# sukui-genomics-cn/hmm_layer

Hardware: AMD Instinct MI355X
Metric: HMM cell-updates/sec (batch x len x states) fwd-bwd, 15-state model (higher is better)
Workload: dtype f32

## Files before the change

hmm_layer_amd/csrc/hmm_engine.hip:

```cpp

#include <hip/hip_runtime.h>
#include <stdint.h>
#include <stdlib.h>
#include <mutex>
#include <type_traits>
#include <vector>
#include "hmm_engine.h"

typedef float f4 __attribute__((ext_vector_type(4)));
typedef int i4 __attribute__((ext_vector_type(4)));

#ifndef HMM_REDUCE_PF
#define HMM_REDUCE_PF 8
#endif
#ifndef HMM_NT_STORE
#define HMM_NT_STORE 1
#endif
#ifndef HMM_PSI
#define HMM_PSI 1
#endif
#ifndef HMM_BWD_FULL
#define HMM_BWD_FULL 0
#endif
#ifndef HMM_FWD_PF2
// ... 46 lines not shown
    int k, b, L, q;
    int NB;
    int T, C;
    int nsub;
    long long nchains;
    int cpw;
    int seq_start;
    int G, gsize;
    size_t o_ops, o_exps, o_prefix, o_llpre, o_suffix, o_lsuf, o_ckpt, o_loglik, o_topo, total;
    size_t o_phi, o_nexact;
    size_t o_flags;
    size_t o_xend, o_rstart;
    size_t o_wtab, o_wlist, o_wcnt, o_dfix;
    size_t o_wshift;
    size_t o_upi;
    size_t o_gops, o_gexps, o_gprefix, o_gllpre, o_gsuffix, o_glsuf;
};

static size_t align_up(size_t x) { return (x + 255) & ~(size_t)255; }
#define PLAN_WIN_STRIDE 34
#define PLAN_WSH_STRIDE 24

static int choose_T(long long NB, int L) {
    {
        const int t = opt(HMM_OPT_CHUNK);
        if (t >= 16 && t <= MAX_T && t % 16 == 0) return t;
    }
    long long t = (NB * (long long)L) / 32768;
    long long tb = 16;
    while (tb * tb * tb * 4 < 9ll * L && tb < MAX_T) tb += 16;
    if (t < tb) t = tb;
    t = ((t + 16 - 1) / 16) * 16;
    if (t < 16) t = 16;
    if (t > MAX_T) t = MAX_T;
    long long lmax = (((long long)L + 16 - 1) / 16) * 16;
    if (t > lmax) t = lmax;
    return (int)t;
}

static int make_plan(int op, int k, int b, int L, int q, Plan *p, int T_fixed = 0) {
    if (k < 1 || b < 1 || L < 1 || q < 1) return HMM_ERR_BAD_SHAPE;
    if (q > QP) return HMM_ERR_Q_UNSUPPORTED;
    if ((long long)k * b > (1ll << 30) / 64) return HMM_ERR_BAD_SHAPE;
    p->k = k; p->b = b; p->L = L; p->q = q;
    p->NB = k * b;
    p->T = T_fixed ? T_fixed : choose_T(p->NB, L);
    p->C = (L + p->T - 1) / p->T;
    p->nsub = p->T / SUB;
    p->nchains = (long long)p->NB * p->C;
    p->cpw = 16;
    p->seq_start = 1;
    size_t off = 0;
    p->o_ops = off;    off = align_up(off + (size_t)p->nchains * QP * QP * sizeof(float));
    p->o_exps = off;   off = align_up(off + (size_t)p->nchains * QP * sizeof(int));
    p->o_prefix = off; off = align_up(off + (size_t)p->nchains * QP * sizeof(float));
    p->o_llpre = off;  off = align_up(off + (size_t)p->nchains * sizeof(double));
    p->o_suffix = off; off = align_up(off + (size_t)p->nchains * QP * sizeof(float));
    p->o_lsuf = off;   off = align_up(off + (size_t)p->nchains * sizeof(double));
    p->o_loglik = off; off = align_up(off + (size_t)p->NB * sizeof(double));
    p->o_topo = off;   off = align_up(off + (size_t)p->k * sizeof(int));
    p->o_phi = off;    off = align_up(off + (size_t)p->nchains * sizeof(float));
    p->o_nexact = off; off = align_up(off + sizeof(int));
    p->o_flags = off;  off = align_up(off + (size_t)p->NB * sizeof(int));
    p->o_xend = off;   off = align_up(off + (size_t)p->nchains * QP * sizeof(float));
    p->o_rstart = off; off = align_up(off + (size_t)p->nchains * QP * sizeof(float));
    p->o_wtab = off;   off = align_up(off + (size_t)p->NB * PLAN_WIN_STRIDE * sizeof(int));
    p->o_wlist = off;  off = align_up(off + (size_t)p->NB * sizeof(int));
    p->o_wcnt = off;   off = align_up(off + 4 * sizeof(int));
    p->o_dfix = off;   off = align_up(off + (size_t)p->NB * sizeof(double));
    p->o_wshift = off; off = align_up(off + ((op == HMM_OP_FORWARD || op == HMM_OP_BACKWARD) ? (size_t)p->NB * PLAN_WSH_STRIDE * sizeof(double) : 0));
    p->o_upi = off;    off = align_up(off + (size_t)p->k * p->q * sizeof(float));
    p->G = 0; p->gsize = 0;
    if (p->C >= SCAN2_MIN_C) {
        int gs = 1;
        while (gs * gs < p->C) ++gs;
        p->gsize = gs;
        p->G = (p->C + gs - 1) / gs;
    }
    const size_t ng = (size_t)p->NB * (p->G > 0 ? p->G : 1);
    p->o_gops = off;    off = align_up(off + ng * QP * QP * sizeof(float));
    p->o_gexps = off;   off = align_up(off + ng * QP * sizeof(int));
    p->o_gprefix = off; off = align_up(off + ng * QP * sizeof(float));
    p->o_gllpre = off;  off = align_up(off + ng * sizeof(double));
    p->o_gsuffix = off; off = align_up(off + ng * QP * sizeof(float));
    p->o_glsuf = off;   off = align_up(off + ng * sizeof(double));
    p->o_ckpt = off;
    if (op == HMM_OP_POSTERIOR) {
        const size_t scan_rows = (size_t)(((long long)p->b * p->C + 15) / 16) * 16 * p->nsub;
        const size_t exact_rows = (size_t)((p->b + 15) / 16) * 16 * (size_t)(((p->L + 15) / 16) * 16 / SUB);
        off = align_up(off + (size_t)p->k * (scan_rows > exact_rows ? scan_rows : exact_rows) * QP * sizeof(float));
    }
    p->total = off;
    return HMM_OK;
}

static int make_xplan(const Plan &p, Plan *x) {
    *x = p;
    x->T = ((p.L + 15) / 16) * 16;
    x->C = 1;
    x->nsub = x->T / SUB;
    x->nchains = p.NB;
    x->G = 0; x->gsize = 0;
    const long long seq_bytes = (long long)x->T * p.q * (long long)sizeof(float);
    x->cpw = 16 * seq_bytes < (1ll << 31) - 4096 ? 16 : 1;
    if (opt(HMM_OPT_EXACT) == HMM_EXACT_ALWAYS_NARROW) x->cpw = 1;
    if (seq_bytes >= (1ll << 31) - 4096) return HMM_ERR_BAD_SHAPE;
    return HMM_OK;
}


__device__ __forceinline__ f4 mfma4(const float (&a)[4], f4 x) {
    const f4 z = {0.f, 0.f, 0.f, 0.f};
    f4 d = __builtin_amdgcn_mfma_f32_16x16x4f32(a[0], x.x, z, 0, 0, 0);
    d = __builtin_amdgcn_mfma_f32_16x16x4f32(a[1], x.y, d, 0, 0, 0);
    d = __builtin_amdgcn_mfma_f32_16x16x4f32(a[2], x.z, d, 0, 0, 0);
    d = __builtin_amdgcn_mfma_f32_16x16x4f32(a[3], x.w, d, 0, 0, 0);
    return d;
}

__device__ __forceinline__ f4 mfma4v(f4 a, f4 x, f4 c) {
    c = __builtin_amdgcn_mfma_f32_16x16x4f32(a.x, x.x, c, 0, 0, 0);
    c = __builtin_amdgcn_mfma_f32_16x16x4f32(a.y, x.y, c, 0, 0, 0);
    c = __builtin_amdgcn_mfma_f32_16x16x4f32(a.z, x.z, c, 0, 0, 0);
    c = __builtin_amdgcn_mfma_f32_16x16x4f32(a.w, x.w, c, 0, 0, 0);
    return c;
}

__device__ __forceinline__ void swap16(float &a, float &b) {
    asm("s_nop 1\n\tv_permlane16_swap_b32_e32 %0, %1" : "+v"(a), "+v"(b));
}
__device__ __forceinline__ void swap32(float &a, float &b) {
    asm("s_nop 1\n\tv_permlane32_swap_b32_e32 %0, %1" : "+v"(a), "+v"(b));
}
__device__ __forceinline__ float col_sum(float v) {
    float a = v, b = v;
    swap16(a, b);
    a += b; b = a;
    swap32(a, b);
    return a + b;
}
__device__ __forceinline__ float col_max(float v) {
    float a = v, b = v;
    swap16(a, b);
    a = fmaxf(a, b); b = a;
    swap32(a, b);
    return fmaxf(a, b);
}
__device__ __forceinline__ float hsum(f4 v) { return (v.x + v.y) + (v.z + v.w); }
__device__ __forceinline__ float hmax(f4 v) { return fmaxf(fmaxf(v.x, v.y), fmaxf(v.z, v.w)); }

__device__ __forceinline__ __amdgpu_buffer_rsrc_t make_rsrc(const void *base, unsigned long long bytes) {
    unsigned n = bytes > 0xFFFFFFF0ull ? 0xFFFFFFF0u : (unsigned)bytes;
    return __builtin_amdgcn_make_buffer_rsrc((void *)base, 0, (int)n, 0x00020000);
}
template <int N>
__device__ __forceinline__ void ld_rows(__amdgpu_buffer_rsrc_t r, int voff, int rowb, f4 (&e)[N]) {
#pragma unroll
    for (int s = 0; s < N; ++s)
        e[s] = __builtin_bit_cast(f4, __builtin_amdgcn_raw_buffer_load_b128(r, voff + s * rowb, 0, HMM_LD_AUX));
}

struct Bounds { f4 lo, hi; };
__device__ __forceinline__ Bounds make_bounds(int g, int q, float eps) {
    Bounds bd;
    const float inf = __builtin_inff();
    bd.lo.x = (4 * g + 0 < q) ? eps : 0.f;  bd.hi.x = (4 * g + 0 < q) ? inf : 0.f;
    bd.lo.y = (4 * g + 1 < q) ? eps : 0.f;  bd.hi.y = (4 * g + 1 < q) ? inf : 0.f;
    bd.lo.z = (4 * g + 2 < q) ? eps : 0.f;  bd.hi.z = (4 * g + 2 < q) ? inf : 0.f;
    bd.lo.w = (4 * g + 3 < q) ? eps : 0.f;  bd.hi.w = (4 * g + 3 < q) ? inf : 0.f;
    return bd;
}
__device__ __forceinline__ f4 clampE(f4 e, const Bounds &bd) {
    f4 r;
    r.x = __builtin_amdgcn_fmed3f(e.x, bd.lo.x, bd.hi.x);
    r.y = __builtin_amdgcn_fmed3f(e.y, bd.lo.y, bd.hi.y);
    r.z = __builtin_amdgcn_fmed3f(e.z, bd.lo.z, bd.hi.z);
    r.w = __builtin_amdgcn_fmed3f(e.w, bd.lo.w, bd.hi.w);
    return r;
}
__device__ __forceinline__ f4 fmax4(f4 v, float s) {
    f4 r = {fmaxf(v.x, s), fmaxf(v.y, s), fmaxf(v.z, s), fmaxf(v.w, s)};
    return r;
}
__device__ __forceinline__ f4 sel4(bool c, f4 a, f4 b) { return c ? a : b; }

__device__ __forceinline__ void load_A(const float *A, int q, int g, int n, float (&af)[4], float (&ab)[4]) {
#pragma unroll
    for (int kk = 0; kk < 4; ++kk) {
        int s = 4 * g + kk;
        bool ok = (s < q) && (n < q);
        af[kk] = ok ? A[s * q + n] : 0.f;
        ab[kk] = ok ? A[n * q + s] : 0.f;
    }
}


__device__ __forceinline__ void reduce_chain(const float *__restrict__ A, const float *__restrict__ E,
                                             float *__restrict__ ops, int *__restrict__ exps,
                                             const int *__restrict__ topo, const Plan &p, float eps, long long chain) {
    const int lane = threadIdx.x & 63, g = lane >> 4, n = lane & 15;
    const int seq = (int)(chain / p.C), c = (int)(chain - (long long)seq * p.C);
    const int m = seq / p.b;
    if (topo && topo[m] != 0) return;
    const int t0 = c * p.T;
    const int len = min(p.T, p.L - t0);
    const int q = p.q;

    float af[4], ab[4];
    load_A(A + (size_t)m * q * q, q, g, n, af, ab);
    const Bounds bd = make_bounds(g, q, eps);

    const float *base = E + ((size_t)seq * p.L + t0) * q;
    const __amdgpu_buffer_rsrc_t rs = make_rsrc(base, (unsigned long long)len * q * sizeof(float));
    const int rowb = q * (int)sizeof(float);
    int voff = g * 16;

    f4 X;
    X.x = (4 * g + 0 == n) ? 1.f : 0.f;
    X.y = (4 * g + 1 == n) ? 1.f : 0.f;
    X.z = (4 * g + 2 == n) ? 1.f : 0.f;
    X.w = (4 * g + 3 == n) ? 1.f : 0.f;
    int ex = 0;

    auto rescale = [&](f4 &V) {
        float s = col_sum(hsum(V));
        int xe = __builtin_amdgcn_frexp_expf(s);
        float sc = __builtin_amdgcn_ldexpf(1.0f, -xe);
        V = V * sc;
        ex += xe;
    };

    int t = 0;
    if (c == 0 && p.seq_start) {
        f4 e0[1];
        ld_rows<1>(rs, voff, rowb, e0);
        X = X * clampE(e0[0], bd);
        rescale(X);
        voff += rowb;
        t = 1;
    }
    constexpr int PF = HMM_REDUCE_PF;
    f4 en[PF];
    ld_rows<PF>(rs, voff, rowb, en);
    for (; t < len; t += PF) {
        f4 ec[PF];
#pragma unroll
        for (int u = 0; u < PF; ++u) ec[u] = en[u];
        voff += PF * rowb;
        ld_rows<PF>(rs, voff, rowb, en);
#pragma unroll
        for (int u = 0; u < PF; ++u) {
            if (t + u < len) {
                X = mfma4(af, X) * clampE(ec[u], bd);
                rescale(X);
            }
        }
    }
    float *o = ops + (size_t)chain * QP * QP;
    o[(4 * g + 0) * QP + n] = X.x;
    o[(4 * g + 1) * QP + n] = X.y;
    o[(4 * g + 2) * QP + n] = X.z;
    o[(4 * g + 3) * QP + n] = X.w;
    if (g == 0) exps[(size_t)chain * QP + n] = ex;
}

__global__ __launch_bounds__(256) void k_reduce(const float *__restrict__ A, const float *__restrict__ E,
                                                float *__restrict__ ops, int *__restrict__ exps,
                                                const int *__restrict__ topo, Plan p, float eps) {
    const long long stride = (long long)gridDim.x * 4;
    for (long long chain = (long long)blockIdx.x * 4 + __builtin_amdgcn_readfirstlane(threadIdx.x >> 6);
         chain < p.nchains; chain += stride)
        reduce_chain(A, E, ops, exps, topo, p, eps, chain);
}



struct TopoGene15 {
    static constexpr int Q = 15, NE = 23, ID = 1;
    static constexpr int start[Q + 1] = {0, 2, 4, 6, 8, 10, 13, 15, 16, 17, 18, 19, 20, 21, 22, 23};
    static constexpr int src[NE] = {0, 14, 8, 1, 9, 2, 10, 3, 11, 6, 7, 4, 12, 5, 13, 0, 4, 5, 6, 1, 2, 3, 5};
};
struct TopoGene7 {
    static constexpr int Q = 7, NE = 15, ID = 2;
    static constexpr int start[Q + 1] = {0, 2, 4, 6, 8, 11, 13, 15};
    static constexpr int src[NE] = {0, 6, 4, 1, 5, 2, 6, 3, 0, 6, 3, 4, 1, 5, 2};
};

struct TopoGene29 {
    static constexpr int Q = 29, NE = 45, ID = 3;
    static constexpr int start[Q + 1] = {0, 3, 5, 7, 9, 11, 13, 15, 17, 19, 22, 25, 27, 29, 30, 31, 32, 33, 34, 35, 36,
                                         37, 38, 39, 40, 41, 42, 43, 44, 45};
    static constexpr int src[NE] = {0, 27, 28, 15, 1, 16, 2, 17, 3, 18, 4, 19, 5, 20, 6, 21, 11, 22, 12, 13, 7, 23, 14,
                                    8, 24, 9, 25, 10, 26, 0, 0, 7, 8, 9, 10, 11, 12, 1, 2, 3, 4, 5, 6, 9, 10};
};

template <class T>
__host__ __device__ constexpr int out_degree(int i) {
    int n = 0;
    for (int e = 0; e < T::NE; ++e) n += (T::src[e] == i) ? 1 : 0;
    return n;
}
#define TOPO_UNIT 16
template <class T>
__device__ __forceinline__ bool edge_in(int i, int j) {
    bool ok = false;
    for (int e = T::start[j]; e < T::start[j + 1]; ++e) ok = ok || (T::src[e] == i);
    return ok;
}

#define TOPO_EXACT 255
__global__ __launch_bounds__(64) void k_topo_check(const float *__restrict__ A, int *__restrict__ topo, int k, int q,
                                                   int force_dense, int exact_mode, float eps, int *__restrict__ nexact,
                                                   int *__restrict__ wcnt = nullptr) {
    const int m = blockIdx.x;
    const float *Am = A + (size_t)m * q * q;
    if (m == 0 && threadIdx.x == 0) *nexact = 0;
    if (m == 0 && threadIdx.x < 4 && wcnt) wcnt[threadIdx.x] = 0;
    bool exact = exact_mode == HMM_EXACT_ALWAYS || exact_mode == HMM_EXACT_ALWAYS_NARROW;
    if (exact_mode == HMM_EXACT_AUTO) {
        int row = 0;
        if ((int)threadIdx.x < q)
            for (int j = 0; j < q; ++j) row |= (Am[threadIdx.x * q + j] > eps) ? (1 << j) : 0;
        for (int it = 0; it < 8; ++it) {
            int nr = 0;
            for (int j = 0; j < q; ++j) {
                const int rj = __builtin_amdgcn_readlane(row, j);
                nr |= ((row >> j) & 1) ? rj : 0;
            }
            row = nr;
        }
        const bool notfull = (int)threadIdx.x < q && row != (1 << q) - 1;
        exact = __ballot(notfull) != 0ull;
    }
    if (exact) {
        if (threadIdx.x == 0) topo[m] = TOPO_EXACT;
        return;
    }
    bool bad15 = q != TopoGene15::Q, bad7 = q != TopoGene7::Q;
    bool nonunit15 = false, nonunit7 = false;
    if (!force_dense && (!bad15 || !bad7))
        for (int e = threadIdx.x; e < q * q; e += 64) {
            const float a = Am[e];
            const int i = e / q, j = e - i * q;
            if (!bad15) {
                const bool in = edge_in<TopoGene15>(i, j);
                bad15 = a != 0.f && !in;
                nonunit15 = nonunit15 || (in && a != 1.0f && out_degree<TopoGene15>(i) == 1);
            }
            if (!bad7) {
                const bool in = edge_in<TopoGene7>(i, j);
                bad7 = a != 0.f && !in;
                nonunit7 = nonunit7 || (in && a != 1.0f && out_degree<TopoGene7>(i) == 1);
            }
        }
    const bool any15 = __ballot(bad15) != 0ull, any7 = __ballot(bad7) != 0ull;
    const bool nu15 = __ballot(nonunit15) != 0ull, nu7 = __ballot(nonunit7) != 0ull;
    if (threadIdx.x == 0) {
        int id = force_dense ? 0 : (!any15 ? TopoGene15::ID : (!any7 ? TopoGene7::ID : 0));
        if (id == TopoGene15::ID && !nu15) id |= TOPO_UNIT;
        if (id == TopoGene7::ID && !nu7) id |= TOPO_UNIT;
        topo[m] = id;
    }
}

#define SP_TILE 16

#ifndef HMM_RS_AHEAD
#define HMM_RS_AHEAD 0
#endif
#ifndef HMM_RS_UNI
#define HMM_RS_UNI 1
#endif
#ifndef HMM_POST_BLOCK
#define HMM_POST_BLOCK 16
#endif
#ifndef HMM_RS_SUM2
#define HMM_RS_SUM2 1
#endif
#ifndef HMM_RS_WPE
#define HMM_RS_WPE 4
#endif
#if HMM_RS_WPE
#define RS_ATTR __attribute__((amdgpu_waves_per_eu(HMM_RS_WPE, HMM_RS_WPE)))
#else
#define RS_ATTR
#endif
template <class T> struct RsCfg {
    static constexpr int W = T::Q <= 16 ? 16 : 32;
    static constexpr int CPW = 64 / W;
    static constexpr int PIECES = SP_TILE * T::Q / 4;
    static constexpr int RPC = (PIECES + 63) / 64;
    typedef float Lds[2][CPW][SP_TILE * W + 16];
};

template <class T, bool UNIT, bool UNI>
__device__ __forceinline__ void reduce_sparse_wave(const float *__restrict__ A, const float *__restrict__ E,
                                                   float *__restrict__ ops, int *__restrict__ exps, const Plan &p,
                                                   float eps, typename RsCfg<T>::Lds &ldsw, long long wchain0,
                                                   bool mine, int m, long long chain, int c) {
    constexpr int Q = T::Q, W = RsCfg<T>::W, CPW = RsCfg<T>::CPW, RPC = RsCfg<T>::RPC;
    const int lane = threadIdx.x & 63, cl = lane / W, kc = lane % W;
    const int t0 = c * p.T;
    const int len = mine ? min(p.T, p.L - t0) : 0;
    const bool first = (c == 0) && p.seq_start;

    float a[T::NE];
    {
        const float *Am = A + (size_t)(UNI ? __builtin_amdgcn_readfirstlane(m) : m) * Q * Q;
#pragma unroll
        for (int j = 0; j < Q; ++j)
#pragma unroll
            for (int e = T::start[j]; e < T::start[j + 1]; ++e) a[e] = Am[T::src[e] * Q + j];
    }

    const int seq0 = (int)(wchain0 / p.C), c0 = (int)(wchain0 - (long long)seq0 * p.C);
    const long long row0 = (long long)seq0 * p.L + (long long)c0 * p.T;
    const unsigned long long total = (unsigned long long)p.NB * p.L * Q * sizeof(float);
    const __amdgpu_buffer_rsrc_t rs = make_rsrc(E + row0 * Q, total - (unsigned long long)row0 * Q * sizeof(float));
    constexpr int PIECES = RsCfg<T>::PIECES;
    static_assert(SP_TILE * Q % 4 == 0, "tile must be a whole number of 16-byte pieces");
    int coff[CPW];
#pragma unroll
    for (int j = 0; j < CPW; ++j) {
        long long ch = wchain0 + j;
        if (ch >= p.nchains) ch = wchain0;
        const long long sq = ch / p.C;
        const long long rw = sq * p.L + (ch - sq * p.C) * (long long)p.T;
        coff[j] = (int)((rw - row0) * Q * (long long)sizeof(float));
    }
    int loff[RPC][4];
#pragma unroll
    for (int rr = 0; rr < RPC; ++rr)
#pragma unroll
        for (int u = 0; u < 4; ++u) {
            const int idx = 4 * (rr * 64 + lane) + u;
            loff[rr][u] = (idx / Q) * W + (idx % Q);
        }
    for (int i = lane; i < 2 * CPW * (SP_TILE * W + 16); i += 64) (&ldsw[0][0][0])[i] = 0.f;

    f4 r[CPW * RPC];
    auto fetch = [&](int tile) {
#pragma unroll
        for (int j = 0; j < CPW; ++j)
#pragma unroll
            for (int rr = 0; rr < RPC; ++rr)
                r[j * RPC + rr] = __builtin_bit_cast(f4, __builtin_amdgcn_raw_buffer_load_b128(
                    rs, coff[j] + tile * (SP_TILE * Q * 4) + (rr * 64 + lane) * 16, 0, 0));
    };
    auto stage = [&](int buf) {
#pragma unroll
        for (int rr = 0; rr < RPC; ++rr) {
            if (rr * 64 + lane < PIECES) {
#pragma unroll
                for (int j = 0; j < CPW; ++j) {
                    float *dst = &ldsw[buf][j][0];
                    const f4 v = r[j * RPC + rr];
                    dst[loff[rr][0]] = fmaxf(v.x, eps);
                    dst[loff[rr][1]] = fmaxf(v.y, eps);
                    dst[loff[rr][2]] = fmaxf(v.z, eps);
                    dst[loff[rr][3]] = fmaxf(v.w, eps);
                }
            }
        }
    };

    float x[Q], pend[Q];
#pragma unroll
    for (int j = 0; j < Q; ++j) { x[j] = (j == kc) ? 1.f : 0.f; pend[j] = 1.f; }
    int ex = 0;
    float cs = (kc < Q) ? 1.f : 0.f;
    auto deferred = [](int j) constexpr { return UNIT && out_degree<T>(j) == 1; };

    bool risk = false;
    auto rescale = [&]() {
        risk = risk || (kc < Q && cs < 0x1p-100f);
        int xe = max(__builtin_amdgcn_frexp_expf(cs), -100);
        float sc = __builtin_amdgcn_ldexpf(1.0f, -xe);
#pragma unroll
        for (int j = 0; j < Q; ++j) x[j] *= sc;
        cs *= sc;
        ex += xe;
    };

    auto column_sum = [&]() {
        float s = 0.f;
#pragma unroll
        for (int j = 0; j < Q; ++j) s += deferred(j) ? x[j] * pend[j] : x[j];
        return s;
    };
    auto finish = [&]() {
        cs = kc < Q ? column_sum() : 0.f;
        rescale();
        float *o = ops + (size_t)chain * W * W;
#pragma unroll
        for (int j = 0; j < Q; ++j) o[j * W + kc] = (kc < Q) ? (deferred(j) ? x[j] * pend[j] : x[j]) : 0.f;
#pragma unroll
        for (int j = Q; j < W; ++j) o[j * W + kc] = 0.f;
        static_assert(Q < W, "the exponent row's last lane is a pad lane");
        const unsigned long long rb = __builtin_amdgcn_ballot_w64(risk) >> (W == 64 ? 0 : W * cl);
        const bool chain_risk = (W == 64 ? rb : (rb & ((1ull << (W & 63)) - 1ull))) != 0ull;
        exps[(size_t)chain * W + kc] = (kc < Q) ? ex : ((kc == W - 1 && chain_risk) ? 1 : 0);
    };
    auto step = [&](const float (&e)[Q], auto sumc) {
        constexpr bool SUM = decltype(sumc)::value;
        float y[Q];
#pragma unroll
        for (int j = 0; j < Q; ++j) {
            float acc = 0.f;
#pragma unroll
            for (int ed = T::start[j]; ed < T::start[j + 1]; ++ed) {
                const int i = T::src[ed];
                const float w = deferred(i) ? pend[i] : a[ed];
                acc = (ed == T::start[j]) ? w * x[i] : fmaf(w, x[i], acc);
            }
            y[j] = acc;
        }
        float s = 0.f;
#pragma unroll
        for (int j = 0; j < Q; ++j) {
            if (SUM) s = fmaf(y[j], e[j], s);
            if (deferred(j)) { x[j] = y[j]; pend[j] = e[j]; }
            else x[j] = y[j] * e[j];
        }
        if (SUM) {
            if (W >= 32) {
                const unsigned long long keep = __builtin_amdgcn_ballot_w64(kc < Q && !(s < cs * 0x1p-45f));
                const unsigned long long mine = W == 64 ? ~0ull : (((1ull << (W & 63)) - 1ull) << (W * cl));
                risk = risk || (keep & mine) == 0ull;
            }
            cs = s;
            const unsigned cb = __builtin_bit_cast(unsigned, cs) - 1u;
            if (__builtin_amdgcn_ballot_w64(cb < 0x2B800000u - 1u) != 0) rescale();
        }
    };

    auto ldrow = [&](const float *rowp, float (&r)[Q]) {
#pragma unroll
        for (int v = 0; v + 4 <= Q; v += 4) {
            const f4 t = *reinterpret_cast<const f4 *>(rowp + v);
            r[v] = t.x; r[v + 1] = t.y; r[v + 2] = t.z; r[v + 3] = t.w;
        }
        constexpr int R0 = Q & ~3;
        if constexpr (Q - R0 == 3) {
            typedef float f3 __attribute__((ext_vector_type(3)));
            const f3 t = *reinterpret_cast<const f3 *>(rowp + R0);
            r[R0] = t.x; r[R0 + 1] = t.y; r[R0 + 2] = t.z;
        } else if constexpr (Q - R0 == 2) {
            typedef float f2 __attribute__((ext_vector_type(2)));
            const f2 t = *reinterpret_cast<const f2 *>(rowp + R0);
            r[R0] = t.x; r[R0 + 1] = t.y;
        } else if constexpr (Q - R0 == 1) {
            r[R0] = rowp[R0];
        }
    };

    const int ntiles = p.T / SP_TILE;
    const int last = len - 1;
    const bool ragged = __builtin_amdgcn_ballot_w64(mine && len != p.T) != 0;
    auto tile_steps = [&](auto checked, int tile, int buf) {
        constexpr bool CHECK = decltype(checked)::value;
        const float *tp = &ldsw[buf][cl][0];
        constexpr bool AHEAD = W == 16 && HMM_RS_AHEAD;
        float c[Q], nx[AHEAD ? Q : 1];
        ldrow(tp, c);
        if constexpr (AHEAD) ldrow(tp + W, nx);
        if (tile == 0) {
            float xs[Q];
#pragma unroll
            for (int j = 0; j < Q; ++j) xs[j] = x[j];
            step(c, std::true_type());
            if (first) {
                const float e0 = tp[kc < Q ? kc : 0];
#pragma unroll
                for (int j = 0; j < Q; ++j) { x[j] = xs[j] * e0; pend[j] = 1.f; }
                cs = (kc < Q) ? e0 : 0.f;
                ex = 0;
                rescale();
            }
        } else {
            step(c, std::integral_constant<bool, !HMM_RS_SUM2>());
        }
        if (CHECK) { if (__builtin_amdgcn_ballot_w64(tile * SP_TILE == last) != 0) { if (tile * SP_TILE == last) finish(); } }
        auto one = [&](int sidx, auto sumc) {
            if constexpr (AHEAD) {
#pragma unroll
                for (int u = 0; u < Q; ++u) c[u] = nx[u];
                if (sidx + 1 < SP_TILE) ldrow(tp + (sidx + 1) * W, nx);
            } else {
                ldrow(tp + sidx * W, c);
            }
            step(c, sumc);
            if (CHECK) {
                const int t = tile * SP_TILE + sidx;
                if (__builtin_amdgcn_ballot_w64(t == last) != 0) { if (t == last) finish(); }
            }
        };
#pragma unroll
        for (int sidx = 1; sidx < SP_TILE; sidx += 2) {
            one(sidx, std::true_type());
            if (sidx + 1 < SP_TILE) one(sidx + 1, std::integral_constant<bool, !HMM_RS_SUM2>());
        }
    };
    fetch(0);
    if (ragged) {
        for (int tile = 0; tile < ntiles; ++tile) {
            stage(tile & 1);
            if (tile + 1 < ntiles) fetch(tile + 1);
            tile_steps(std::true_type(), tile, tile & 1);
        }
    } else {
        for (int tile = 0; tile < ntiles; ++tile) {
            stage(tile & 1);
            if (tile + 1 < ntiles) fetch(tile + 1);
            tile_steps(std::false_type(), tile, tile & 1);
        }
        if (mine) finish();
    }
}

template <class T, bool MIXED>
__device__ __forceinline__ void reduce_sparse_block(const float *__restrict__ A, const float *__restrict__ E,
                                                    float *__restrict__ ops, int *__restrict__ exps,
                                                    const int *__restrict__ topo, const Plan &p, float eps) {
    __shared__ __attribute__((aligned(16))) typename RsCfg<T>::Lds lds[4];
    const int w = __builtin_amdgcn_readfirstlane(threadIdx.x >> 6);
    const int lane = threadIdx.x & 63, cl = lane / RsCfg<T>::W;
    const long long wchain0 = ((long long)blockIdx.x * 4 + w) * RsCfg<T>::CPW;
    if (wchain0 >= p.nchains) return;
    const long long chain = wchain0 + cl;
    const bool inrange = chain < p.nchains;
    const long long chn = inrange ? chain : wchain0;
    const int seq = (int)(chn / p.C), c = (int)(chn - (long long)seq * p.C);
    const int m = seq / p.b;
    const int tp = topo[m];
    const bool mine = inrange && (tp & (TOPO_UNIT - 1)) == T::ID && tp != TOPO_EXACT;
    const unsigned long long mmask = __builtin_amdgcn_ballot_w64(mine);
    if (mmask == 0) return;
    const bool unit = __builtin_amdgcn_ballot_w64(mine && (tp & TOPO_UNIT)) == mmask;
    const bool uni = HMM_RS_UNI && __builtin_amdgcn_ballot_w64(m != __builtin_amdgcn_readfirstlane(m)) == 0ull;
    if (uni == MIXED) return;
    if (unit) reduce_sparse_wave<T, true, !MIXED>(A, E, ops, exps, p, eps, lds[w], wchain0, mine, m, chain, c);
    else reduce_sparse_wave<T, false, !MIXED>(A, E, ops, exps, p, eps, lds[w], wchain0, mine, m, chain, c);
}

template <class T, bool MIXED = false>
__global__ __launch_bounds__(256) RS_ATTR void k_reduce_sparse(const float *__restrict__ A, const float *__restrict__ E,
                                                       float *__restrict__ ops, int *__restrict__ exps,
                                                       const int *__restrict__ topo, Plan p, float eps) {
    reduce_sparse_block<T, MIXED>(A, E, ops, exps, topo, p, eps);
}
template <class T, bool MIXED = false>
__global__ __launch_bounds__(256) void k_reduce_sparse_wide(const float *__restrict__ A, const float *__restrict__ E,
                                                            float *__restrict__ ops, int *__restrict__ exps,
                                                            const int *__restrict__ topo, Plan p, float eps) {
    reduce_sparse_block<T, MIXED>(A, E, ops, exps, topo, p, eps);
}


template <class Op>
__device__ __forceinline__ int row_allreduce_i(int v, Op op) {
    v = op(v, __builtin_amdgcn_update_dpp(v, v, 0xB1, 0xF, 0xF, false));
    v = op(v, __builtin_amdgcn_update_dpp(v, v, 0x4E, 0xF, 0xF, false));
    v = op(v, __builtin_amdgcn_update_dpp(v, v, 0x141, 0xF, 0xF, false));
    v = op(v, __builtin_amdgcn_update_dpp(v, v, 0x140, 0xF, 0xF, false));
    return v;
}
__device__ __forceinline__ float row_sum_f(float x) {
    int v = __builtin_bit_cast(int, x);
    auto add = [](int a, int b) { return __builtin_bit_cast(int, __builtin_bit_cast(float, a) + __builtin_bit_cast(float, b)); };
    return __builtin_bit_cast(float, row_allreduce_i(v, add));
}
__device__ __forceinline__ int row_max_i(int x) {
    return row_allreduce_i(x, [](int a, int b) { return a > b ? a : b; });
}
__device__ __forceinline__ float lane_bcast(float x, int srclane) {
    return __builtin_bit_cast(float, __builtin_amdgcn_readlane(__builtin_bit_cast(int, x), srclane));
}
template <int K>
__device__ __forceinline__ float row_bcast_f(float x) {
    return __builtin_bit_cast(float, __builtin_amdgcn_update_dpp(0, __builtin_bit_cast(int, x), 0x150 + K, 0xF, 0xF, false));
}
__device__ __forceinline__ float row_dot16(const float (&c)[16], float v) {
    float a0 = 0.f, a1 = 0.f;
    a0 = fmaf(c[0], row_bcast_f<0>(v), a0);   a1 = fmaf(c[1], row_bcast_f<1>(v), a1);
    a0 = fmaf(c[2], row_bcast_f<2>(v), a0);   a1 = fmaf(c[3], row_bcast_f<3>(v), a1);
    a0 = fmaf(c[4], row_bcast_f<4>(v), a0);   a1 = fmaf(c[5], row_bcast_f<5>(v), a1);
    a0 = fmaf(c[6], row_bcast_f<6>(v), a0);   a1 = fmaf(c[7], row_bcast_f<7>(v), a1);
    a0 = fmaf(c[8], row_bcast_f<8>(v), a0);   a1 = fmaf(c[9], row_bcast_f<9>(v), a1);
    a0 = fmaf(c[10], row_bcast_f<10>(v), a0); a1 = fmaf(c[11], row_bcast_f<11>(v), a1);
    a0 = fmaf(c[12], row_bcast_f<12>(v), a0); a1 = fmaf(c[13], row_bcast_f<13>(v), a1);
    a0 = fmaf(c[14], row_bcast_f<14>(v), a0); a1 = fmaf(c[15], row_bcast_f<15>(v), a1);
    return a0 + a1;
}

__global__ __launch_bounds__(128) void k_scan(const float *__restrict__ pi, const float *__restrict__ ops,
                                             const int *__restrict__ exps, float *__restrict__ prefix,
                                             double *__restrict__ llpre, float *__restrict__ suffix,
                                             double *__restrict__ lsuf, double *__restrict__ loglik,
                                             const int *__restrict__ topo, Plan p, float eps,
                                             const float *__restrict__ pre_in = nullptr,
                                             const double *__restrict__ ll_in = nullptr,
                                             const float *__restrict__ suf_in = nullptr,
                                             const double *__restrict__ ls_in = nullptr) {
    const int seq = blockIdx.x;
    const int lane = threadIdx.x & 63;
    const int dir = __builtin_amdgcn_readfirstlane(threadIdx.x >> 6);
    const int n = lane & 15;
    const int q = p.q, C = p.C;
    const int m = seq / p.b;
    const size_t chain0 = (size_t)seq * C;
    if (lane >= 16) return;
    if (topo[m] == TOPO_EXACT) return;
    if (dir == 0) {
        float praw = pre_in ? pre_in[(size_t)seq * QP + n] : ((n < q) ? pi[(size_t)m * q + n] : 0.f);
        float a = pre_in ? praw : ((n < q) ? fmaxf(praw, eps) : 0.f);
        double ll = ll_in ? ll_in[seq] : 0.0;
        prefix[chain0 * QP + n] = praw;
        if (n == 0) llpre[chain0] = ll;
        const f4 *row = reinterpret_cast<const f4 *>(ops + chain0 * QP * QP + n * QP);
        f4 r0 = row[0], r1 = row[1], r2 = row[2], r3 = row[3];
        int xe = exps[chain0 * QP + n];
        for (int c = 0; c < C; ++c) {
            const f4 q0 = r0, q1 = r1, q2 = r2, q3 = r3;
            const int xec = xe;
            if (c + 1 < C) {
                const f4 *nx = reinterpret_cast<const f4 *>(ops + (chain0 + c + 1) * QP * QP + n * QP);
                r0 = nx[0]; r1 = nx[1]; r2 = nx[2]; r3 = nx[3];
                xe = exps[(chain0 + c + 1) * QP + n];
            }
            int we = (a > 0.f) ? __builtin_amdgcn_frexp_expf(a) + xec : -(1 << 28);
            const int emax = row_max_i(we);
            int sh = xec - emax;
            sh = sh < -300 ? -300 : sh;
            float w = __builtin_amdgcn_ldexpf(a, sh);
            float acc = 0.f;
            float xr[16] = {q0.x, q0.y, q0.z, q0.w, q1.x, q1.y, q1.z, q1.w, q2.x, q2.y, q2.z, q2.w, q3.x, q3.y, q3.z, q3.w};
#pragma unroll
            for (int kk = 0; kk < 16; ++kk) acc = fmaf(xr[kk], lane_bcast(w, kk), acc);
            const float S = row_sum_f(acc);
            a = acc / S;
            ll += (double)__logf(S) + (double)emax * LN2;
            if (c + 1 < C) {
                prefix[(chain0 + c + 1) * QP + n] = a;
                if (n == 0) llpre[chain0 + c + 1] = ll;
            }
        }
        if (n == 0) loglik[seq] = ll;
    } else {
        float v = suf_in ? suf_in[(size_t)seq * QP + n] : ((n < q) ? 1.f : 0.f);
        double lb = ls_in ? ls_in[seq] : 0.0;
        float col[16];
        int xe = 0;
        if (C > 1) {
            const float *X = ops + (chain0 + C - 1) * QP * QP;
#pragma unroll
            for (int j = 0; j < 16; ++j) col[j] = X[j * QP + n];
            xe = exps[(chain0 + C - 1) * QP + n];
        }
        for (int c = C - 1; c >= 0; --c) {
            suffix[(chain0 + c) * QP + n] = v;
            if (n == 0) lsuf[chain0 + c] = lb;
            if (c == 0) break;
            float cc[16];
#pragma unroll
            for (int j = 0; j < 16; ++j) cc[j] = col[j];
            const int xec = xe;
            if (c - 1 > 0) {
                const float *X = ops + (chain0 + c - 1) * QP * QP;
#pragma unroll
                for (int j = 0; j < 16; ++j) col[j] = X[j * QP + n];
                xe = exps[(chain0 + c - 1) * QP + n];
            }
            float u = 0.f;
#pragma unroll
            for (int j = 0; j < 16; ++j) u = fmaf(cc[j], lane_bcast(v, j), u);
            int we = (u > 0.f) ? __builtin_amdgcn_frexp_expf(u) + xec : -(1 << 28);
            const int emax = row_max_i(we);
            int sh = xec - emax;
            sh = sh < -300 ? -300 : sh;
            v = __builtin_amdgcn_ldexpf(u, sh);
            lb += (double)emax * LN2;
        }
    }
}

__device__ __forceinline__ int col_max_i(int v) {
    float a = __builtin_bit_cast(float, v), b2 = a;
    swap16(a, b2);
    v = max(__builtin_bit_cast(int, a), __builtin_bit_cast(int, b2));
    a = __builtin_bit_cast(float, v); b2 = a;
    swap32(a, b2);
    return max(__builtin_bit_cast(int, a), __builtin_bit_cast(int, b2));
}

__global__ __launch_bounds__(256) void k_scan_compose(const float *__restrict__ ops, const int *__restrict__ exps,
                                                      float *__restrict__ gops, int *__restrict__ gexps,
                                                      const int *__restrict__ topo, Plan p) {
    const long long wv = (long long)blockIdx.x * 4 + __builtin_amdgcn_readfirstlane(threadIdx.x >> 6);
    if (wv >= (long long)p.NB * p.G) return;
    const int lane = threadIdx.x & 63, g = lane >> 4, n = lane & 15;
    const int seq = (int)(wv / p.G), grp = (int)(wv - (long long)seq * p.G);
    if (topo[seq / p.b] == TOPO_EXACT) return;
    const int c0 = grp * p.gsize, c1 = min(p.C, c0 + p.gsize);
    f4 X = {4 * g + 0 == n ? 1.f : 0.f, 4 * g + 1 == n ? 1.f : 0.f, 4 * g + 2 == n ? 1.f : 0.f, 4 * g + 3 == n ? 1.f : 0.f};
    int ex = 0;
    const size_t chb = (size_t)seq * p.C;
    f4 an[SCAN_PF];
    i4 en[SCAN_PF];
#pragma unroll
    for (int u = 0; u < SCAN_PF; ++u) {
        const int c = min(c0 + u, c1 - 1);
        an[u] = *reinterpret_cast<const f4 *>(ops + (chb + c) * QP * QP + n * QP + 4 * g);
        en[u] = *reinterpret_cast<const i4 *>(exps + (chb + c) * QP + 4 * g);
    }
    for (int cb = c0; cb < c1; cb += SCAN_PF)
#pragma unroll
      for (int u = 0; u < SCAN_PF; ++u) {
        const int c = cb + u;
        if (c >= c1) break;
        const f4 a4 = an[u];
        const i4 e4 = en[u];
        if (c + SCAN_PF < c1) {
            an[u] = *reinterpret_cast<const f4 *>(ops + (chb + c + SCAN_PF) * QP * QP + n * QP + 4 * g);
            en[u] = *reinterpret_cast<const i4 *>(exps + (chb + c + SCAN_PF) * QP + 4 * g);
        }
        int we = -(1 << 28);
        we = X.x > 0.f ? max(we, __builtin_amdgcn_frexp_expf(X.x) + e4.x) : we;
        we = X.y > 0.f ? max(we, __builtin_amdgcn_frexp_expf(X.y) + e4.y) : we;
        we = X.z > 0.f ? max(we, __builtin_amdgcn_frexp_expf(X.z) + e4.z) : we;
        we = X.w > 0.f ? max(we, __builtin_amdgcn_frexp_expf(X.w) + e4.w) : we;
        const int emax = col_max_i(we);
        f4 W;
        W.x = __builtin_amdgcn_ldexpf(X.x, max(e4.x - emax, -300));
        W.y = __builtin_amdgcn_ldexpf(X.y, max(e4.y - emax, -300));
        W.z = __builtin_amdgcn_ldexpf(X.z, max(e4.z - emax, -300));
        W.w = __builtin_amdgcn_ldexpf(X.w, max(e4.w - emax, -300));
        const float af[4] = {a4.x, a4.y, a4.z, a4.w};
        X = mfma4(af, W);
        const float sden = col_sum(hsum(X));
        const int xe = __builtin_amdgcn_frexp_expf(sden);
        X = X * __builtin_amdgcn_ldexpf(1.0f, -xe);
        ex += emax + xe;
    }
    float *o = gops + (size_t)wv * QP * QP;
    o[(4 * g + 0) * QP + n] = X.x;
    o[(4 * g + 1) * QP + n] = X.y;
    o[(4 * g + 2) * QP + n] = X.z;
    o[(4 * g + 3) * QP + n] = X.w;
    if (g == 0) gexps[(size_t)wv * QP + n] = ex;
}

__global__ __launch_bounds__(128) void k_scan_inner(const float *__restrict__ ops, const int *__restrict__ exps,
                                                   const float *__restrict__ gprefix, const double *__restrict__ gllpre,
                                                   const float *__restrict__ gsuffix, const double *__restrict__ glsuf,
                                                   float *__restrict__ prefix, double *__restrict__ llpre,
                                                   float *__restrict__ suffix, double *__restrict__ lsuf,
                                                   const int *__restrict__ topo, Plan p, float eps) {
    const int lane = threadIdx.x & 63;
    const int dir = __builtin_amdgcn_readfirstlane(threadIdx.x >> 6);
    const int n = lane & 15;
    const int q = p.q;
    const long long blk = (long long)blockIdx.x * 4 + (lane >> 4);
    bool valid = blk < (long long)p.NB * p.G;
    const long long bl = valid ? blk : 0;
    const int seq = (int)(bl / p.G), grp = (int)(bl - (long long)seq * p.G);
    valid = valid && topo[seq / p.b] != TOPO_EXACT;
    const int c0 = grp * p.gsize, c1 = min(p.C, c0 + p.gsize);
    const size_t chain0 = (size_t)seq * p.C;
    int hops = valid ? c1 - 1 - c0 : 0;
    for (int o = 32; o > 0; o >>= 1) hops = max(hops, __shfl_xor(hops, o));
    if (dir == 0) {
        const float pin = valid ? gprefix[(size_t)bl * QP + n] : 0.f;
        float a = (grp == 0 && p.seq_start) ? ((n < q) ? fmaxf(pin, eps) : 0.f) : pin;
        double ll = valid ? gllpre[bl] : 0.0;
        if (valid) {
            prefix[(chain0 + c0) * QP + n] = pin;
            if (n == 0) llpre[chain0 + c0] = ll;
// ... 1522 lines not shown
```

Measured before the change: 256.0 billion.

## Eliminate pass-through states in sparse reduce via second-order recurrence

Pass-through states (one in-edge, one out-edge) are dropped from the per-step state vector. Each is represented by its pending emission times the previous step's live source value, kept in an extra register array. The pass-through transition weight is folded into the emissions when they are staged in LDS, so each step does matrix work only over the live states (7 of 15 in the gene model). A second change reads the trailing 3-float row remainder as one 16-byte load using the pad float. The price is extra registers for the lagged vector and more complex handling of the first step.

```diff
diff --git a/hmm_layer_amd/csrc/hmm_engine.hip b/hmm_layer_amd/csrc/hmm_engine.hip
--- a/hmm_layer_amd/csrc/hmm_engine.hip
+++ b/hmm_layer_amd/csrc/hmm_engine.hip
@@ -372,6 +372,34 @@
 }
 #define TOPO_UNIT 16
 template <class T>
+__host__ __device__ constexpr bool passthrough(int j) {
+    return T::start[j + 1] - T::start[j] == 1 && out_degree<T>(j) == 1;
+}
+template <class T>
+__host__ __device__ constexpr int pt_src(int p) { return T::src[T::start[p]]; }
+template <class T>
+__host__ __device__ constexpr int pt_dst(int p) {
+    for (int j = 0; j < T::Q; ++j)
+        for (int e = T::start[j]; e < T::start[j + 1]; ++e)
+            if (T::src[e] == p) return j;
+    return -1;
+}
+template <class T>
+__host__ __device__ constexpr int n_passthrough() {
+    int n = 0;
+    for (int j = 0; j < T::Q; ++j) n += passthrough<T>(j) ? 1 : 0;
+    return n;
+}
+template <class T>
+__host__ __device__ constexpr bool passthrough_between_live() {
+    for (int p = 0; p < T::Q; ++p)
+        if (passthrough<T>(p) && (passthrough<T>(pt_src<T>(p)) || passthrough<T>(pt_dst<T>(p)))) return false;
+    return true;
+}
+static_assert(n_passthrough<TopoGene15>() == 8 && passthrough_between_live<TopoGene15>(), "15-state gene model: 7 live states");
+static_assert(n_passthrough<TopoGene29>() == 16 && passthrough_between_live<TopoGene29>(), "29-state gene model: 13 live states");
+static_assert(n_passthrough<TopoGene7>() == 0, "the 7-state model has no pass-through state");
+template <class T>
 __device__ __forceinline__ bool edge_in(int i, int j) {
     bool ok = false;
     for (int e = T::start[j]; e < T::start[j + 1]; ++e) ok = ok || (T::src[e] == i);
@@ -447,6 +475,12 @@
 #ifndef HMM_RS_SUM2
 #define HMM_RS_SUM2 1
 #endif
+#ifndef HMM_RS_ORDER2
+#define HMM_RS_ORDER2 1
+#endif
+#ifndef HMM_RS_ROW128
+#define HMM_RS_ROW128 1
+#endif
 #ifndef HMM_RS_WPE
 #define HMM_RS_WPE 4
 #endif
@@ -469,6 +503,9 @@
                                                    float eps, typename RsCfg<T>::Lds &ldsw, long long wchain0,
                                                    bool mine, int m, long long chain, int c) {
     constexpr int Q = T::Q, W = RsCfg<T>::W, CPW = RsCfg<T>::CPW, RPC = RsCfg<T>::RPC;
+    constexpr bool O2 = HMM_RS_ORDER2 && UNIT && UNI && n_passthrough<T>() > 0;
+    static_assert(!O2 || passthrough_between_live<T>(), "a pass-through state between two live states");
+    auto live = [](int j) constexpr { return !O2 || !passthrough<T>(j); };
     const int lane = threadIdx.x & 63, cl = lane / W, kc = lane % W;
     const int t0 = c * p.T;
     const int len = mine ? min(p.T, p.L - t0) : 0;
@@ -506,6 +543,20 @@
             const int idx = 4 * (rr * 64 + lane) + u;
             loff[rr][u] = (idx / Q) * W + (idx % Q);
         }
+    float smul[O2 ? RPC : 1][4];
+    if constexpr (O2) {
+#pragma unroll
+        for (int rr = 0; rr < RPC; ++rr)
+#pragma unroll
+            for (int u = 0; u < 4; ++u) {
+                const int st = (4 * (rr * 64 + lane) + u) % Q;
+                float mv = 1.f;
+#pragma unroll
+                for (int pp = 0; pp < Q; ++pp)
+                    if (passthrough<T>(pp)) mv = (st == pp) ? a[T::start[pp]] : mv;
+                smul[rr][u] = mv;
+            }
+    }
     for (int i = lane; i < 2 * CPW * (SP_TILE * W + 16); i += 64) (&ldsw[0][0][0])[i] = 0.f;
 
     f4 r[CPW * RPC];
@@ -525,21 +576,42 @@
                 for (int j = 0; j < CPW; ++j) {
                     float *dst = &ldsw[buf][j][0];
                     const f4 v = r[j * RPC + rr];
-                    dst[loff[rr][0]] = fmaxf(v.x, eps);
-                    dst[loff[rr][1]] = fmaxf(v.y, eps);
-                    dst[loff[rr][2]] = fmaxf(v.z, eps);
-                    dst[loff[rr][3]] = fmaxf(v.w, eps);
+                    if constexpr (O2) {
+                        dst[loff[rr][0]] = fmaxf(v.x, eps) * smul[rr][0];
+                        dst[loff[rr][1]] = fmaxf(v.y, eps) * smul[rr][1];
+                        dst[loff[rr][2]] = fmaxf(v.z, eps) * smul[rr][2];
+                        dst[loff[rr][3]] = fmaxf(v.w, eps) * smul[rr][3];
+                    } else {
+                        dst[loff[rr][0]] = fmaxf(v.x, eps);
+                        dst[loff[rr][1]] = fmaxf(v.y, eps);
+                        dst[loff[rr][2]] = fmaxf(v.z, eps);
+                        dst[loff[rr][3]] = fmaxf(v.w, eps);
+                    }
                 }
             }
         }
     };
 
-    float x[Q], pend[Q];
-#pragma unroll
-    for (int j = 0; j < Q; ++j) { x[j] = (j == kc) ? 1.f : 0.f; pend[j] = 1.f; }
+    float x[Q], pend[Q], xb[O2 ? Q : 1];
+    auto flight_src = [&](int i) {
+        bool f = false;
+#pragma unroll
+        for (int pp = 0; pp < Q; ++pp)
+            if (passthrough<T>(pp) && pt_src<T>(pp) == i) f = f || (kc == pp);
+        return f;
+    };
+#pragma unroll
+    for (int j = 0; j < Q; ++j) {
+        x[j] = (j == kc) ? 1.f : 0.f;
+        pend[j] = 1.f;
+        if constexpr (O2) {
+            pend[j] = x[j];
+            xb[j] = flight_src(j) ? 1.f : 0.f;
+        }
+    }
     int ex = 0;
     float cs = (kc < Q) ? 1.f : 0.f;
-    auto deferred = [](int j) constexpr { return UNIT && out_degree<T>(j) == 1; };
+    auto deferred = [](int j) constexpr { return !O2 && UNIT && out_degree<T>(j) == 1; };
 
     bool risk = false;
     auto rescale = [&]() {
@@ -547,15 +619,29 @@
         int xe = max(__builtin_amdgcn_frexp_expf(cs), -100);
         float sc = __builtin_amdgcn_ldexpf(1.0f, -xe);
 #pragma unroll
-        for (int j = 0; j < Q; ++j) x[j] *= sc;
+        for (int j = 0; j < Q; ++j) {
+            if (live(j)) x[j] *= sc;
+            if constexpr (O2) { if (live(j)) xb[j] *= sc; }
+        }
         cs *= sc;
         ex += xe;
     };
 
+    auto entry = [&](int j) {
+        if constexpr (O2) return live(j) ? x[j] : pend[j] * xb[pt_src<T>(j)];
+        else return deferred(j) ? x[j] * pend[j] : x[j];
+    };
     auto column_sum = [&]() {
         float s = 0.f;
-#pragma unroll
-        for (int j = 0; j < Q; ++j) s += deferred(j) ? x[j] * pend[j] : x[j];
+        if constexpr (O2) {
+#pragma unroll
+            for (int j = 0; j < Q; ++j) if (live(j)) s += x[j];
+#pragma unroll
+            for (int j = 0; j < Q; ++j) if (!live(j)) s = fmaf(pend[j], xb[pt_src<T>(j)], s);
+        } else {
+#pragma unroll
+            for (int j = 0; j < Q; ++j) s += entry(j);
+        }
         return s;
     };
     auto finish = [&]() {
@@ -563,7 +649,7 @@
         rescale();
         float *o = ops + (size_t)chain * W * W;
 #pragma unroll
-        for (int j = 0; j < Q; ++j) o[j * W + kc] = (kc < Q) ? (deferred(j) ? x[j] * pend[j] : x[j]) : 0.f;
+        for (int j = 0; j < Q; ++j) o[j * W + kc] = (kc < Q) ? entry(j) : 0.f;
 #pragma unroll
         for (int j = Q; j < W; ++j) o[j * W + kc] = 0.f;
         static_assert(Q < W, "the exponent row's last lane is a pad lane");
@@ -574,23 +660,50 @@
     auto step = [&](const float (&e)[Q], auto sumc) {
         constexpr bool SUM = decltype(sumc)::value;
         float y[Q];
-#pragma unroll
-        for (int j = 0; j < Q; ++j) {
-            float acc = 0.f;
-#pragma unroll
-            for (int ed = T::start[j]; ed < T::start[j + 1]; ++ed) {
-                const int i = T::src[ed];
-                const float w = deferred(i) ? pend[i] : a[ed];
-                acc = (ed == T::start[j]) ? w * x[i] : fmaf(w, x[i], acc);
-            }
-            y[j] = acc;
-        }
         float s = 0.f;
-#pragma unroll
-        for (int j = 0; j < Q; ++j) {
-            if (SUM) s = fmaf(y[j], e[j], s);
-            if (deferred(j)) { x[j] = y[j]; pend[j] = e[j]; }
-            else x[j] = y[j] * e[j];
+        if constexpr (O2) {
+#pragma unroll
+            for (int j = 0; j < Q; ++j) {
+                if (!live(j)) continue;
+                float acc = 0.f;
+                bool any = false;
+#pragma unroll
+                for (int pass = 0; pass < 2; ++pass)
+#pragma unroll
+                    for (int ed = T::start[j]; ed < T::start[j + 1]; ++ed) {
+                        const int i = T::src[ed];
+                        if (live(i) != (pass == 0)) continue;
+                        const float w = live(i) ? a[ed] : pend[i];
+                        const float v = live(i) ? x[i] : xb[pt_src<T>(i)];
+                        acc = any ? fmaf(w, v, acc) : w * v;
+                        any = true;
+                    }
+                y[j] = acc;
+            }
+#pragma unroll
+            for (int j = 0; j < Q; ++j) {
+                if (live(j)) { xb[j] = x[j]; x[j] = y[j] * e[j]; }
+                else pend[j] = e[j];
+            }
+            if (SUM) s = column_sum();
+        } else {
+#pragma unroll
+            for (int j = 0; j < Q; ++j) {
+                float acc = 0.f;
+#pragma unroll
+                for (int ed = T::start[j]; ed < T::start[j + 1]; ++ed) {
+                    const int i = T::src[ed];
+                    const float w = deferred(i) ? pend[i] : a[ed];
+                    acc = (ed == T::start[j]) ? w * x[i] : fmaf(w, x[i], acc);
+                }
+                y[j] = acc;
+            }
+#pragma unroll
+            for (int j = 0; j < Q; ++j) {
+                if (SUM) s = fmaf(y[j], e[j], s);
+                if (deferred(j)) { x[j] = y[j]; pend[j] = e[j]; }
+                else x[j] = y[j] * e[j];
+            }
         }
         if (SUM) {
             if (W >= 32) {
@@ -611,7 +724,11 @@
             r[v] = t.x; r[v + 1] = t.y; r[v + 2] = t.z; r[v + 3] = t.w;
         }
         constexpr int R0 = Q & ~3;
-        if constexpr (Q - R0 == 3) {
+        if constexpr (Q - R0 == 3 && HMM_RS_ROW128) {
+            static_assert(R0 + 4 <= W, "the pad float belongs to the row");
+            const f4 t = *reinterpret_cast<const f4 *>(rowp + R0);
+            r[R0] = t.x; r[R0 + 1] = t.y; r[R0 + 2] = t.z;
+        } else if constexpr (Q - R0 == 3) {
             typedef float f3 __attribute__((ext_vector_type(3)));
             const f3 t = *reinterpret_cast<const f3 *>(rowp + R0);
             r[R0] = t.x; r[R0 + 1] = t.y; r[R0 + 2] = t.z;
@@ -637,12 +754,18 @@
         if (tile == 0) {
             float xs[Q];
 #pragma unroll
-            for (int j = 0; j < Q; ++j) xs[j] = x[j];
+            for (int j = 0; j < Q; ++j) xs[j] = O2 ? (j == kc ? 1.f : 0.f) : x[j];
+            float e0 = 1.f;
+            if constexpr (O2) { if (first && mine && kc < Q) e0 = fmaxf(E[(chain / p.C) * (long long)p.L * Q + kc], eps); }
             step(c, std::true_type());
             if (first) {
-                const float e0 = tp[kc < Q ? kc : 0];
-#pragma unroll
-                for (int j = 0; j < Q; ++j) { x[j] = xs[j] * e0; pend[j] = 1.f; }
+                if constexpr (!O2) e0 = tp[kc < Q ? kc : 0];
+#pragma unroll
+                for (int j = 0; j < Q; ++j) {
+                    x[j] = xs[j] * e0;
+                    pend[j] = 1.f;
+                    if constexpr (O2) { pend[j] = x[j]; xb[j] = flight_src(j) ? 1.f : 0.f; }
+                }
                 cs = (kc < Q) ? e0 : 0.f;
                 ex = 0;
                 rescale();
```

Measured after the change: 265.6 billion, median of 6. +3.7%, better.
